# SinOncology/BreakID

Hardware: AMD Instinct MI355X
Metric: M reads/s clustered+split-scanned (higher is better)
Workload: dtype int32/u8 (+f64 sd replay)

## Files before the change

breakid_amd/csrc/lanes.hip:

```cpp
#include <algorithm>
#include <atomic>
#include <chrono>
#include <cmath>
#include <cstdio>
#include <numeric>
#include <thread>
#include <dirent.h>

#include "lanes.h"

static int g_hw_queues_at_init = 0;
void stage_set_hw_queues(int n) { g_hw_queues_at_init = n; }

static bool sort_service_on()
{
  static const bool on = !(getenv("BREAKID_SORT_SERVICE") && atoi(getenv("BREAKID_SORT_SERVICE")) == 0);
  return on;
}
constexpr int LANE_STREAMS_MAX = 4;
constexpr int SVC_STAGE_QUEUES = LANE_STREAMS_MAX + 3;
static bool lane_service(int fast) { return sort_service_on() && fast && g_hw_queues_at_init >= SVC_STAGE_QUEUES; }
static int stage_queues() { return std::max(1, g_hw_queues_at_init - 1); }
static int lanes_wanted(bool svc)
{
  const char *env = getenv("BREAKID_GROUP_LANES");
  static const int want_svc = env ? atoi(env) : 12;
  if (svc) return want_svc < 1 ? 1 : (want_svc > 26 ? 26 : want_svc);
  static const int want = env ? atoi(env) : std::min(4, stage_queues());
  return want < 1 ? 1 : (want > 26 ? 26 : want);
}
static bool lanes_apply(const StageInput &in, int fast)
{
  static const uint64_t min_pairs = getenv("BREAKID_LANES_MIN_PAIRS") ? strtoull(getenv("BREAKID_LANES_MIN_PAIRS"), nullptr, 10) : (1ull << 20);
  uint32_t large = 0;
  const uint64_t big = std::max<uint64_t>(2, min_pairs >> 6);
  for (uint32_t g = 0; g < in.jr.n_groups && g + 1 < in.gstart_host.size(); ++g) large += in.gstart_host[g + 1] - in.gstart_host[g] >= big ? 1u : 0u;
  const bool yes = lanes_wanted(lane_service(fast)) >= 2 && fast && in.jr.n_groups >= 4 && in.jr.n_pairs >= min_pairs && large >= 2;
  if (yes)
  {
    static bool told = false;
    const int K = lanes_wanted(lane_service(fast));
    if (!told && !lane_service(fast) && K > stage_queues() && bk_debug("lanes"))
    {
      told = true;
      fprintf(stderr, "[breakid] GPU_MAX_HW_QUEUES=%d: the lanes of chromosome-pair groups (bk_mask_and_cluster) and their heap kernels will share hardware queues "
                        "(BREAKID_GROUP_LANES=1: one pass)\n", g_hw_queues_at_init);
    }
  }
  return yes;
}

__global__ void k_svc_probe() {}
static int kfd_compute_queues(int device)
{
  char bus[64] = {0};
  if (hipDeviceGetPCIBusId(bus, (int) sizeof bus, device) != hipSuccess) return -1;
  unsigned dom = 0, b = 0, d = 0, f = 0;
  if (sscanf(bus, "%x:%x:%x.%x", &dom, &b, &d, &f) != 4) return -1;
  const unsigned long want_loc = (b << 8) | (d << 3) | f;
  auto read_file = [](const std::string &path, std::string &out) {
    FILE *fp = fopen(path.c_str(), "r");
    if (!fp) return false;
    char buf[4096];
    const size_t n = fread(buf, 1, sizeof buf - 1, fp);
    fclose(fp);
    buf[n] = 0;
    out = buf;
    return true;
  };
  auto list_dir = [](const std::string &path, std::vector<std::string> &names) {
    DIR *dp = opendir(path.c_str());
    if (!dp) return false;
    while (dirent *e = readdir(dp))
      if (e->d_name[0] != '.') names.push_back(e->d_name);
    closedir(dp);
    return true;
  };
  unsigned long gpu_id = 0;
  {
    std::vector<std::string> nodes;
    if (!list_dir("/sys/class/kfd/kfd/topology/nodes", nodes)) return -1;
    for (const std::string &n : nodes)
    {
      std::string props, id;
      const std::string base = "/sys/class/kfd/kfd/topology/nodes/" + n;
      if (!read_file(base + "/properties", props) || !read_file(base + "/gpu_id", id)) continue;
      unsigned long loc = ~0ul, domain = ~0ul;
      size_t p = props.find("location_id ");
      if (p != std::string::npos) loc = strtoul(props.c_str() + p + 12, nullptr, 10);
      p = props.find("domain ");
      if (p != std::string::npos) domain = strtoul(props.c_str() + p + 7, nullptr, 10);
      if (loc == want_loc && (domain == ~0ul || domain == dom) && strtoul(id.c_str(), nullptr, 10) != 0) gpu_id = strtoul(id.c_str(), nullptr, 10);
// ... 77 lines not shown
    cs.svc_late = 0;
    set(&cs.svc);
  }
  bool reachable(const std::vector<hipStream_t> &streams)
  {
    while (cs.svc_probe.size() < streams.size())
    {
      hipEvent_t e;
      HIP_CHECK(hipEventCreateWithFlags(&e, hipEventDisableTiming));
      cs.svc_probe.push_back(e);
    }
    for (size_t k = 0; k < streams.size(); ++k)
    {
      hipLaunchKernelGGL(k_svc_probe, dim3(1), dim3(64), 0, streams[k]);
      HIP_CHECK(hipEventRecord(cs.svc_probe[k], streams[k]));
    }
    const auto t0 = std::chrono::steady_clock::now();
    auto since = [&] { return std::chrono::duration<double>(std::chrono::steady_clock::now() - t0).count(); };
    bool ok = true;
    for (size_t k = 0; k < streams.size() && ok; ++k)
      for (;;)
      {
        const hipError_t e = hipEventQuery(cs.svc_probe[k]);
        if (e == hipSuccess) break;
        if (e != hipErrorNotReady) throw bk_error(BK_ERR_HIP, std::string("sort service probe: ") + hipGetErrorString(e));
        if (since() > 0.05)
        {
          ok = false;
          break;
        }
      }
    const double took = since();
    if (bk_debug("lanes")) fprintf(stderr, "[lanes] sort service probe: %zu streams in %.3f ms%s\n", streams.size(), took * 1e3, ok ? "" : " (gave up)");
    return ok && took < 0.003;
  }
  void set(SortService *s)
  {
    for (auto &l : cs.lanes)
    {
      l->cb.se.svc = s;
      l->cb.se.svc_slot = 0xFFFFFFFFu;
    }
  }
  void finish()
  {
    if (!on) return;
    on = false;
    set(nullptr);
    hipError_t e = hipStreamSynchronize(st);
    for (auto &l : cs.lanes)
      if (l->st && e == hipSuccess) e = hipStreamSynchronize(l->st);
    cs.svc.stop();
    device_turn.unlock();
    if (e != hipSuccess) throw bk_error(BK_ERR_HIP, std::string("sort service: ") + hipGetErrorString(e));
  }
  ~SvcStage()
  {
    try
    {
      finish();
    }
    catch (const bk_error &)
    {
    }
  }
};

static void snapshot_list(const PairList &L, DevBuf &idx, DevBuf *gof, DevBuf &goff, hipStream_t st)
{
  uint32_t *ii = idx.as<uint32_t>(L.n + 1), *ig = gof ? gof->as<uint32_t>(L.n + 1) : nullptr;
  uint64_t *io = goff.as<uint64_t>((uint64_t) L.ng + 1);
  if (L.n) HIP_CHECK(hipMemcpyAsync(ii, L.idx.get<uint32_t>(), L.n * 4, hipMemcpyDeviceToDevice, st));
  if (L.n && ig) HIP_CHECK(hipMemcpyAsync(ig, L.gof.get<uint32_t>(), L.n * 4, hipMemcpyDeviceToDevice, st));
  if (L.ng) HIP_CHECK(hipMemcpyAsync(io, L.goff.get<uint64_t>(), ((uint64_t) L.ng + 1) * 8, hipMemcpyDeviceToDevice, st));
}
static void cluster_list(const bk_pair *pairs, PairList &L, double w, int fast, DevBuf &cl, ClusterBufs &cb, AhcBufs &ab, hipStream_t st)
{
  if (fast)
    fast_cluster_all(pairs, L, w, cl, cb, st);
  else
    ahc_cluster_all(pairs, L, w, cl, ab, cb, st);
}

using LanePlan = std::vector<int>;
static LanePlan plan_owned(const StageInput &in)
{
  const uint32_t ng = in.jr.n_groups;
  const bool owned_only = !in.own_groups.empty();
  if (owned_only && in.own_groups.size() != ng) throw bk_error(BK_ERR_ARG, "bk_shard_own_groups: group count changed");
  LanePlan p(ng, 0);
  for (uint32_t g = 0; owned_only && g < ng; ++g)
    if (!in.own_groups[g]) p[g] = -1;
  return p;
}
static LanePlan plan_blind(const StageInput &in, int K)
{
  const uint32_t ng = in.jr.n_groups;
  std::vector<uint32_t> order(ng);
  std::iota(order.begin(), order.end(), 0u);
  auto size_of = [&](uint32_t g) { return in.gstart_host[g + 1] - in.gstart_host[g]; };
  std::stable_sort(order.begin(), order.end(), [&](uint32_t a, uint32_t b) { return size_of(a) > size_of(b); });
  constexpr double wexp = 2.0;
  LanePlan p = plan_owned(in);
  std::vector<double> load(K, 0.0);
  for (uint32_t i = 0; i < ng; ++i)
  {
    const uint32_t g = order[i];
    if (p[g] < 0) continue;
    int l = 0;
    for (int k = 1; k < K; ++k)
      if (load[k] < load[l]) l = k;
    load[l] += std::pow((double) size_of(g), wexp);
    p[g] = l;
  }
  return p;
}
static LanePlan plan_observed(const std::vector<uint64_t> &sizes, const std::vector<uint32_t> &hx, const std::vector<uint32_t> &hy, int K)
{
  const uint32_t ng = (uint32_t) sizes.size();
  constexpr double per_pair = 0.001;
  auto heap_cost = [](uint32_t m) { return (double) m + (m > 40947u ? 1.0 * (double) (m - 40947u) : 0.0); };
  std::vector<uint32_t> order(ng);
  std::iota(order.begin(), order.end(), 0u);
  auto chain = [&](uint32_t g) { return heap_cost(hx[g]) + heap_cost(hy[g]); };
  std::stable_sort(order.begin(), order.end(), [&](uint32_t a, uint32_t b) {
    const double ca = chain(a), cb = chain(b);
    return ca != cb ? ca > cb : sizes[a] > sizes[b];
  });
  LanePlan p(ng, 0);
  std::vector<double> mx(K, 0.0), my(K, 0.0), pairs(K, 0.0);
  auto cost = [&](int l) { return mx[l] + my[l] + per_pair * pairs[l]; };
  for (uint32_t g : order)
  {
    int best = 0;
    double best_cost = 0;
    for (int l = 0; l < K; ++l)
    {
      const double c = std::max(mx[l], heap_cost(hx[g])) + std::max(my[l], heap_cost(hy[g])) + per_pair * (pairs[l] + (double) sizes[g]);
      if (l == 0 || c < best_cost || (c == best_cost && cost(l) < cost(best)))
      {
        best = l;
        best_cost = c;
      }
    }
    mx[best] = std::max(mx[best], heap_cost(hx[g]));
    my[best] = std::max(my[best], heap_cost(hy[g]));
    pairs[best] += (double) sizes[g];
    p[g] = best;
  }
  if (bk_debug("lanes"))
    for (int l = 0; l < K; ++l)
    {
      fprintf(stderr, "[lanes] lane %d: max heap x %.0f y %.0f, %.0f pairs, cost %.0f; heavy groups:", l, mx[l], my[l], pairs[l], cost(l));
      for (uint32_t g = 0; g < ng; ++g)
        if (p[g] == l && (hx[g] || hy[g])) fprintf(stderr, " %u(%u,%u)", g, hx[g], hy[g]);
      fprintf(stderr, "\n");
    }
  return p;
}
static uint32_t *upload_drop(const LanePlan &p, int K, DevBuf &buf, hipStream_t st)
{
  const size_t row = p.size() + 1;
  std::vector<uint32_t> drop((size_t) K * row, 0u);
  for (int l = 0; l < K; ++l)
    for (size_t g = 0; g + 1 < row; ++g) drop[(size_t) l * row + g] = p[g] == l ? 0u : 1u;
  uint32_t *d = buf.as<uint32_t>(drop.size() + 1);
  HIP_CHECK(hipMemcpyAsync(d, drop.data(), drop.size() * 4, hipMemcpyHostToDevice, st));
  HIP_CHECK(hipStreamSynchronize(st));
  return d;
}

static void group_lanes(ClusterStage &cs, const StageInput &in, double w, int fast)
{
  const uint32_t ng = in.jr.n_groups;
  static const bool dbg = bk_debug("lanes");
  auto make_lanes = [&](int K, int S) {
    while ((int) cs.lanes.size() < K)
    {
      cs.lanes.emplace_back(new ClusterStage::Lane());
      cs.lanes.back()->cb.max_group_bound = cs.cb().max_group_bound;
    }
    for (int k = 1; k < S; ++k)
      if (!cs.lanes[k]->st) HIP_CHECK(hipStreamCreateWithFlags(&cs.lanes[k]->st, hipStreamNonBlocking));
  };
  bool use_svc = sort_service_on() && fast;
  if (use_svc && !lane_service(fast))
  {
    use_svc = false;
    tell_no_service();
    if (bk_debug("lanes")) fprintf(stderr, "[lanes] %d hardware queues, the sort service needs %d: not started\n", g_hw_queues_at_init, SVC_STAGE_QUEUES);
  }
  int K = lanes_wanted(use_svc);
  int S = use_svc ? std::max(1, std::min(LANE_STREAMS_MAX, K)) : K;
  make_lanes(K, S);
  std::vector<hipStream_t> stage_streams{in.st};
  for (int k = 1; k < S; ++k) stage_streams.push_back(cs.lanes[k]->st);
  SvcStage svc_stage(cs, in.device, in.st, use_svc, in.jr.n_pairs + 2ull * ng + 4096, cs.cb().max_group_bound, stage_streams);
  if (use_svc && !svc_stage.on)
  {
    use_svc = false;
    K = lanes_wanted(false);
    S = K;
    make_lanes(K, S);
  }
  if (!use_svc && bk_debug("lanes"))
  {
    fprintf(stderr, "[lanes] launch path: %d lanes, 1 stream each, %d hardware queues\n", K, g_hw_queues_at_init);
    fprintf(stderr, "[lanes] sorts as task dispatches on the lane streams\n");
  }
  auto lane = [&](int l) -> ClusterStage::Lane & { return *cs.lanes[l]; };
  auto lane_st = [&](int l) { const int k = l % S; return k == 0 ? in.st : cs.lanes[k]->st; };
  uint32_t *drop_base = nullptr;
  auto lane_drop = [&](int l) { return drop_base + (size_t) l * ((size_t) ng + 1); };
  std::vector<std::vector<uint8_t>> keep(K, std::vector<uint8_t>(ng, 0));
  auto upload_plan = [&](const LanePlan &p) {
    for (int l = 0; l < K; ++l)
      for (uint32_t g = 0; g < ng; ++g) keep[l][g] = p[g] == l ? 1 : 0;
    drop_base = upload_drop(p, K, cs.d_drop, in.st);
  };
  auto in_lanes = [&](auto body) {
    std::vector<std::string> err(K);
    std::vector<int> code(K, BK_OK);
    const auto t_start = std::chrono::steady_clock::now();
    auto guarded_body = [&](int l) {
      try
      {
        body(l);
        HIP_CHECK(hipStreamSynchronize(lane_st(l)));
        if (dbg)
          fprintf(stderr, "[lanes] lane %d done after %.2f ms\n", l, std::chrono::duration<double, std::milli>(std::chrono::steady_clock::now() - t_start).count());
      }
      catch (const bk_error &e)
      {
        code[l] = e.code;
        err[l] = e.msg;
      }
    };
    std::vector<std::thread> th;
    for (int l = 1; l < K; ++l)
      th.emplace_back([&, l] {
        (void) hipSetDevice(in.device);
        guarded_body(l);
      });
    guarded_body(0);
    for (std::thread &t : th) t.join();
    for (int l = 0; l < K; ++l)
      if (code[l] != BK_OK) throw bk_error(code[l], err[l]);
  };
  auto merge_all = [&](PairList ClusterStage::Lane::*which, PairList &out, DevBuf *cl_out) {
    std::vector<const PairList *> ls(K);
    std::vector<const uint32_t *> cls(K);
    for (int l = 0; l < K; ++l)
    {
      ls[l] = &(lane(l).*which);
      cls[l] = lane(l).d_cluster.get<uint32_t>();
    }
    merge_lists_many(ls.data(), cl_out ? cls.data() : nullptr, K, out, cl_out, in.st);
  };
  const bk_pair *pairs = in.jr.pairs;
  auto mask_lane = [&](int l, bool observe) {
    ClusterBufs &cb = lane(l).cb;
    if (observe)
    {
      cb.heavy_x.assign(ng, 0u);
      cb.heavy_y.assign(ng, 0u);
      cb.observe = true;
      cb.se.heavy_all = false;
    }
    remove_isolated_begin(pairs, in.jr.gof, in.jr.gstart, ng, in.jr.n_pairs, w, lane(l).list, cb, lane_st(l), lane_drop(l), in.gstart_host.data(), keep[l].data());
    if (observe) cb.heavy_x.assign(ng, 0u);
    remove_isolated_end(pairs, lane(l).list, cb, lane_st(l));
    if (observe) cb.observe = false;
  };
  auto cluster_lane = [&](int l) {
    PairList &L = lane(l).list, &iso = lane(l).iso;
    iso.n = L.n;
    iso.ng = L.ng;
    snapshot_list(L, iso.idx, &iso.gof, iso.goff, lane_st(l));
    cluster_list(pairs, L, w, fast, lane(l).d_cluster, lane(l).cb, cs.ab, lane_st(l));
  };
  const auto tp0 = std::chrono::steady_clock::now();
  auto phase = [&](const char *what) {
    if (dbg) fprintf(stderr, "[lanes] %s at %.2f ms\n", what, std::chrono::duration<double, std::milli>(std::chrono::steady_clock::now() - tp0).count());
  };
  upload_plan(plan_blind(in, K));
  phase("plan uploaded");
  if (use_svc)
    in_lanes([&](int l) {
      mask_lane(l, false);
      cluster_lane(l);
    });
  else
  {
    in_lanes([&](int l) { mask_lane(l, true); });
    PairList &mid = cs.lane_mid;
    merge_all(&ClusterStage::Lane::list, mid, nullptr);
    std::vector<uint64_t> goff_h((size_t) ng + 1);
    HIP_CHECK(hipMemcpyAsync(goff_h.data(), mid.goff.get<uint64_t>(), ((size_t) ng + 1) * 8, hipMemcpyDeviceToHost, in.st));
    HIP_CHECK(hipStreamSynchronize(in.st));
    std::vector<uint64_t> sizes(ng);
    std::vector<uint32_t> hx(ng, 0u), hy(ng, 0u);
    for (uint32_t g = 0; g < ng; ++g) sizes[g] = goff_h[g + 1] - goff_h[g];
    for (int l = 0; l < K; ++l)
      for (uint32_t g = 0; g < ng; ++g)
      {
        hx[g] = std::max(hx[g], lane(l).cb.heavy_x[g]);
        hy[g] = std::max(hy[g], lane(l).cb.heavy_y[g]);
      }
    upload_plan(plan_observed(sizes, hx, hy, K));
    in_lanes([&](int l) {
      list_subset_ranges(mid, goff_h.data(), keep[l].data(), lane(l).list, lane_st(l));
      cluster_lane(l);
    });
  }
  phase("lanes done");
  svc_stage.finish();
  phase("service stopped");
  if (use_svc && bk_debug("lanes")) fprintf(stderr, "[svc] tasks: %u wide, %u narrow\n", cs.svc.stats[0], cs.svc.stats[1]);
  PairList &iso_m = cs.lane_iso_m;
  merge_all(&ClusterStage::Lane::iso, iso_m, nullptr);
  merge_all(&ClusterStage::Lane::list, cs.list, &cs.d_cluster);
  HIP_CHECK(hipStreamSynchronize(in.st));
  phase("lists merged");
  cs.iso_n = iso_m.n;
  std::swap(cs.iso_idx, iso_m.idx);
  std::swap(cs.iso_goff, iso_m.goff);
}

void ClusterStage::run(const StageInput &in, double w, int fast)
{
  uint64_t mg = 0;
  for (uint32_t g = 0; g < in.jr.n_groups && g + 1 < in.gstart_host.size(); ++g) mg = std::max<uint64_t>(mg, in.gstart_host[g + 1] - in.gstart_host[g]);
  for (auto &l : lanes) l->cb.max_group_bound = mg;
  if (lanes_apply(in, fast))
  {
    in.timed("mask_and_cluster_lanes", [&] { group_lanes(*this, in, w, fast); });
    return;
  }
  SvcStage svc_stage(*this, in.device, in.st, true, in.jr.n_pairs + 2ull * in.jr.n_groups + 4096, cb().max_group_bound, {in.st});
  in.timed("remove_isolated", [&] {
    const uint32_t *drop = in.own_groups.empty() ? nullptr : upload_drop(plan_owned(in), 1, d_drop, in.st);
    remove_isolated_all(in.jr.pairs, in.jr.gof, in.jr.gstart, in.jr.n_groups, in.jr.n_pairs, w, list, cb(), in.st, drop);
  });
  iso_n = list.n;
  snapshot_list(list, iso_idx, nullptr, iso_goff, in.st);
  if (!fast) svc_stage.finish();
  in.timed(fast ? "fast_cluster" : "ahc_cluster", [&] { cluster_list(in.jr.pairs, list, w, fast, d_cluster, cb(), ab, in.st); });
  svc_stage.finish();
}

void ClusterStage::sort_forms(uint64_t out[3]) const
{
  out[0] = out[1] = out[2] = 0;
  for (const auto &l : lanes)
    for (int k = 0; k < 2; ++k) out[k] += l->cb.se.sorts[k];
}

void ClusterStage::debug_sort(int device, hipStream_t st, uint32_t *key, uint32_t *idx, const uint32_t *gof, const uint64_t *goff, uint32_t ng, uint64_t n, uint64_t max_group)
{
  SvcStage svc_stage(*this, device, st, true, n + 2ull * ng + 4096, max_group, {st});
  std_sort_groups(key, idx, gof, goff, ng, n, cb().se, st);
  svc_stage.finish();
}
```

breakid_amd/csrc/sortemu.h:

```cpp
#pragma once
#include "bk_common.h"
#include <vector>
#include <atomic>

struct SortService
{
  DevBuf ctl, slots[2], seq[2], jobs, dbg, pos[2];
  uint32_t pos_cap[2] = {0, 0};
  uint32_t cap[2] = {0, 0};
  hipStream_t st[2] = {nullptr, nullptr}, quit_stream = nullptr, st_copy = nullptr;
  uint32_t *quit_host = nullptr;
  uint32_t *quit_dev = nullptr;
  uint32_t cap32 = 0;
  uint32_t quit_word = 0, starts = 0;
  size_t wide_lds = 0;
  bool running = false;
  std::atomic<uint32_t> next_slot{0};
  uint32_t stats[8] = {};
  void start(uint64_t n_bound, uint64_t max_group, hipStream_t after);
  bool narrow_running(double seconds) const;
  void stop();
  uint32_t new_slot() { return next_slot.fetch_add(1u); }
  ~SortService();
  SortService() = default;
  SortService(const SortService &) = delete;
  SortService &operator=(const SortService &) = delete;
};

struct SortEmuBufs
{
  SortService *svc = nullptr;
  uint32_t svc_slot = 0xFFFFFFFFu, svc_epoch = 0;
  DevBuf heap_scratch, scratch32, scratch32b, rk_a, rk_b, chk_key0, chk_cnt, chk_bad;
  std::vector<uint32_t> *heavy = nullptr;
  bool heavy_all = false;
  DevBuf tj_ctl, tj_jobs, tj_slots[2], tj_seq[2], tj_pos[2], tj_heavy, tj_trace;
  uint32_t tj_cap[2] = {0, 0}, tj_epoch = 0;
  bool tj_ready = false;
  uint64_t sorts[2] = {0, 0};
  SortEmuBufs() = default;
  SortEmuBufs(const SortEmuBufs &) = delete;
  SortEmuBufs &operator=(const SortEmuBufs &) = delete;
};

void std_sort_groups(uint32_t *key, uint32_t *idx, const uint32_t *gof, const uint64_t *goff, uint32_t ng, uint64_t n, SortEmuBufs &b, hipStream_t st);
```

breakid_amd/csrc/sortemu.hip:

```cpp
#include "bk_common.h"
#include "sortemu.h"
#include <vector>
#include <mutex>
#include <algorithm>
#include <cstdio>
#include <chrono>
#include <thread>
#include <cstdlib>

namespace
{
typedef __attribute__((address_space(1))) uint32_t gu32_t;
__device__ __forceinline__ void st_through(uint32_t *p, uint32_t v) { __hip_atomic_store((gu32_t *) p, v, __ATOMIC_RELAXED, __HIP_MEMORY_SCOPE_AGENT); }
constexpr uint32_t FIN_MAX = 2048;
constexpr uint32_t HEAP_BIG_MIN = 4096;

typedef unsigned long long hent;
__device__ __forceinline__ uint32_t hkey(hent e) { return (uint32_t) (e >> 32); }

struct E64
{
  typedef hent T;
  static __device__ __forceinline__ uint32_t key(T e) { return (uint32_t) (e >> 32); }
};
struct E32
{
  typedef uint32_t T;
  static __device__ __forceinline__ uint32_t key(T e) { return e >> 16; }
};

template <class E> struct LdsMemT
{
  typedef typename E::T T;
  T *e;
  static __device__ __forceinline__ uint32_t key(T v) { return E::key(v); }
  __device__ __forceinline__ T ld(uint32_t i) const { return e[i]; }
  __device__ __forceinline__ void st(uint32_t i, T v) const { e[i] = v; }
  __device__ __forceinline__ void step_sync() const { __builtin_amdgcn_wave_barrier(); }
  __device__ __forceinline__ void launch_sync() const { __builtin_amdgcn_wave_barrier(); }
};
template <class E> struct GlbMemT
{
  typedef typename E::T T;
  T *e;
  static __device__ __forceinline__ uint32_t key(T v) { return E::key(v); }
  __device__ __forceinline__ T ld(uint32_t i) const { return e[i]; }
  __device__ __forceinline__ void st(uint32_t i, T v) const { e[i] = v; }
  __device__ __forceinline__ void step_sync() const { asm volatile("s_waitcnt vmcnt(0)" ::: "memory"); }
  __device__ __forceinline__ void launch_sync() const {}
};
typedef LdsMemT<E64> LdsMem;
typedef GlbMemT<E64> GlbMem;

template <class M> __device__ __forceinline__ bool sift_step(const M &mem, uint32_t &hole, uint32_t len, typename M::T v)
{
  typedef typename M::T T;
  const uint32_t right = 2 * (hole + 1), left = right - 1;
  T ec = 0;
  uint32_t c = 0;
  bool has = true;
  if (right < len)
  {
    const T el = mem.ld(left), er = mem.ld(right);
    if (M::key(er) < M::key(el))
    {
      c = left;
      ec = el;
    }
    else
    {
      c = right;
      ec = er;
    }
  }
  else if (left < len)
  {
    c = left;
    ec = mem.ld(left);
  }
  else
    has = false;
  if (has && !(M::key(ec) < M::key(v)))
  {
    mem.st(hole, ec);
// ... 962 lines not shown
        fprintf(stderr, "[svc]   %s workgroups by last state (1 polling, 5 took a task, 9 left):", kind ? "narrow" : "wide");
        for (auto &kv : hist) fprintf(stderr, " %u:%d", kv.first, kv.second);
        fprintf(stderr, "; first ones (state, polls, time of the last poll in 10 ns, how it left 6 error 7 quit 8 timeout):");
        for (uint32_t w = 0; w < 6 && w < n; ++w) fprintf(stderr, " [%u %u %u %u]", d[4 * (w + 4096 * kind)], d[4 * (w + 4096 * kind) + 1], d[4 * (w + 4096 * kind) + 2], d[4 * (w + 4096 * kind) + 3]);
        fprintf(stderr, "\n");
      }
    }
    uint32_t sq[4] = {};
    HIP_CHECK(hipMemcpy(sq, seq[1].get<uint32_t>(), sizeof sq, hipMemcpyDeviceToHost));
    fprintf(stderr, "[svc] tasks %u wide / %u narrow; workgroups started %u / %u, left on their own %u / %u, odd quit words read %u; error %u; wide queue head %u tail %u, narrow queue head %u tail %u (seq %u %u %u %u); job 0: remaining %u done %u heaps %u (longest %u)\n",
            stats[0], stats[1], stats[2], stats[3], stats[4], stats[5], stats[6], h[0], c[0], c[32], c[64], c[96], sq[0], sq[1], sq[2], sq[3], j0.remaining, j0.done, j0.n_heap, j0.max_heap);
  }
  if (h[0]) throw bk_error(h[0] & 2u ? BK_ERR_LIMIT : BK_ERR_HIP, "sort service: task error " + std::to_string(h[0]) + " (2 = ring overflow, 4 = a job timed out, 8 = a cut outside its segment, 16 = a task in the wrong queue, 32 = a node beyond the position lists, 64 = the finisher); first failing task: code " + std::to_string(h[8]) + ", " + std::to_string(h[9]) + " " + std::to_string(h[10]) + " " + std::to_string(h[11]));
}
SortService::~SortService()
{
  if (running)
  {
    running = false;
    if (quit_host && st_copy)
    {
      __atomic_store_n(quit_host, quit_word, __ATOMIC_SEQ_CST);
      (void) hipMemcpyAsync(ctl.get<uint32_t>() + 192, quit_host, 4, hipMemcpyHostToDevice, st_copy);
    }
    if (quit_stream) hipLaunchKernelGGL(k_svc_quit, dim3(1), dim3(1), 0, quit_stream, ctl.get<uint32_t>() + 192, quit_word);
    for (int k = 0; k < 2; ++k)
      if (st[k]) (void) hipStreamSynchronize(st[k]);
    DeferredFrees::end();
  }
  for (int k = 0; k < 2; ++k)
    if (st[k]) (void) hipStreamDestroy(st[k]);
  if (st_copy) (void) hipStreamDestroy(st_copy);
  if (quit_host) (void) hipHostFree(quit_host);
}

static void window_sorts(uint32_t *key, uint32_t *idx, const uint32_t *gof, uint32_t n, hipStream_t st);

static void std_sort_groups_svc(uint32_t *key, uint32_t *idx, const uint32_t *gof, const uint64_t *goff, uint32_t ng, uint32_t n, SortEmuBufs &b, hipStream_t st)
{
  SortService &S = *b.svc;
  if (b.svc_slot == 0xFFFFFFFFu)
  {
    b.svc_slot = S.new_slot();
    if (b.svc_slot >= SVC_MAX_JOBS) throw bk_error(BK_ERR_LIMIT, "sort service: more than 64 callers");
  }
  SvcJob d = {};
  d.key = key;
  d.idx = idx;
  d.hscratch = b.heap_scratch.as<hent>((uint64_t) n + HEAP_PAD);
  d.scratch32 = b.scratch32.as<uint32_t>((uint64_t) n + HEAP_PAD);
  d.scratch32b = b.scratch32b.as<uint32_t>((uint64_t) n + HEAP_PAD);
  d.rka = b.rk_a.as<unsigned long long>((uint64_t) n + HEAP_PAD);
  d.rkb = b.rk_b.as<unsigned long long>((uint64_t) n + HEAP_PAD);
  d.epoch = (b.svc_epoch++ % 0xFFFFFu) + 1u;
  const SvcParams P = svc_params(S);
  hipLaunchKernelGGL(k_svc_submit, dim3(1), dim3(256), 0, st, P, d, b.svc_slot, goff, ng);
  HIP_CHECK(hipGetLastError());
  {
    volatile const uint32_t *done = S.quit_host + SVC_H_DONE + b.svc_slot, *err = S.quit_host + SVC_H_ERROR;
    const auto t0 = std::chrono::steady_clock::now();
    for (uint32_t spins = 0; *done != d.epoch; ++spins)
    {
      if (*err != 0u)
        throw bk_error(BK_ERR_HIP, "sort service: a task failed (error " + std::to_string(*err) + "; first failing task: code " + std::to_string(err[1]) + ", " + std::to_string(err[2]) + " " + std::to_string(err[3]) + " " + std::to_string(err[4]) + ")");
      if ((spins & 1023u) == 1023u)
      {
        if (std::chrono::duration<double>(std::chrono::steady_clock::now() - t0).count() > 20.0) throw bk_error(BK_ERR_HIP, "sort service: a job did not finish");
        std::this_thread::yield();
      }
      else
        __builtin_ia32_pause();
    }
  }
  if (bk_debug("svc"))
  {
    SvcJob j;
    HIP_CHECK(hipMemcpy(&j, S.jobs.get<SvcJob>() + b.svc_slot, sizeof j, hipMemcpyDeviceToHost));
    fprintf(stderr, "[svc] slot %u sort %u: %u elements in %u groups; partitions and finisher done after %.3f ms, job after %.3f ms; %u elements in heaps, the longest %u, the heap that ended last %u elements in %.3f ms\n", b.svc_slot,
            b.svc_epoch, n, ng, (double) (j.t_parts - j.t_submit) * 1e-5, (double) (j.t_done - j.t_submit) * 1e-5, j.n_heap, j.max_heap, (uint32_t) j.last_heap, (double) (j.last_heap >> 32) * 1e-5);
  }
  window_sorts(key, idx, gof, n, st);
}

static void std_sort_groups_tasks(uint32_t *key, uint32_t *idx, const uint32_t *gof, const uint64_t *goff, uint32_t ng, uint32_t n, SortEmuBufs &b, hipStream_t st, const uint32_t *key0)
{
  static size_t dyn_lds = 0;
  static uint32_t cap32 = 0;
  static std::once_flag once;
  std::call_once(once, [] {
    const WideLds w = wide_lds_split(reinterpret_cast<const void *>(k_sort_job));
    dyn_lds = w.dyn_lds;
    cap32 = w.cap32;
    if (dyn_lds < SJ_TEAMS * SJ_TEAM_LDS) throw bk_error(BK_ERR_HIP, "k_sort_job: the narrow teams do not fit the LDS");
    HIP_CHECK(hipFuncSetAttribute(reinterpret_cast<const void *>(k_sort_job), hipFuncAttributeMaxDynamicSharedMemorySize, (int) dyn_lds));
  });
  std::vector<uint64_t> go((size_t) ng + 1);
  HIP_CHECK(hipMemcpyAsync(go.data(), goff, go.size() * 8, hipMemcpyDeviceToHost, st));
  HIP_CHECK(hipStreamSynchronize(st));
  uint64_t max_group = 0;
  for (uint32_t g = 0; g < ng; ++g) max_group = std::max<uint64_t>(max_group, go[g + 1] - go[g]);
  const uint32_t n_wide = std::min<uint32_t>(SJ_MAX_WIDE, std::max<uint32_t>(1, cdiv(n, 1u << 16)));
  const uint32_t n_narrow = std::min<uint32_t>(SJ_MAX_NARROW, std::max<uint32_t>(1, cdiv(n, 1u << 16)));
  SjParams S = {};
  SvcParams &P = S.P;
  {
    auto pow2 = [](uint64_t v) {
      uint32_t c = 1024;
      while (c < v && c < (1u << 30)) c <<= 1;
      return c;
    };
    const uint32_t want[2] = {pow2((uint64_t) n / HEAP_BIG_MIN + 4096), pow2((uint64_t) n / 16 + 4096)};
    for (int k = 0; k < 2; ++k)
      if (want[k] > b.tj_cap[k])
      {
        b.tj_cap[k] = want[k];
        b.tj_ready = false;
      }
    uint32_t *ctl = b.tj_ctl.as<uint32_t>(SJ_C_WORDS);
    for (int k = 0; k < 2; ++k)
    {
      P.q[k].head = ctl + 64 * k;
      P.q[k].tail = ctl + 64 * k + 32;
      P.q[k].slots = b.tj_slots[k].as<SvcTask>(b.tj_cap[k]);
      P.q[k].seq = b.tj_seq[k].as<uint32_t>(b.tj_cap[k]);
      P.q[k].mask = b.tj_cap[k] - 1;
      P.q[k].release = 1u;
    }
    P.error = ctl + SJ_C_ERROR;
    P.stats = ctl + SJ_C_STATS;
    P.quit_d = ctl + SJ_C_QUIT;
    P.host = ctl + SJ_C_HOST;
    P.jobs = b.tj_jobs.as<SvcJob>(SVC_MAX_JOBS);
    P.cap32 = cap32;
    P.quit_word = 0u;
    P.timeout_ticks = SJ_TIMEOUT_TICKS;
    P.pos_cap[0] = (uint32_t) std::max<uint64_t>(max_group, SVC_WIDE_MIN) + 64;
    P.pos_cap[1] = SVC_WIDE_MIN + 64;
    P.pos[0] = b.tj_pos[0].as<uint32_t>(2ull * P.pos_cap[0] * n_wide);
    P.pos[1] = b.tj_pos[1].as<uint32_t>(2ull * P.pos_cap[1] * n_narrow * SJ_TEAMS);
    P.dbg = nullptr;
    S.n_wide = n_wide;
    S.live = ctl + SJ_C_LIVE;
    S.gof = gof;
    S.heavy_min = b.heavy_all ? FIN_MAX : HEAP_RANKED_MIN;
    if (b.heavy)
    {
      S.heavy = b.tj_heavy.as<uint32_t>(ng);
      HIP_CHECK(hipMemsetAsync(S.heavy, 0, (size_t) ng * 4, st));
    }
  }
  static const bool dbg = bk_debug("svc");
  if (dbg) S.trace = b.tj_trace.as<unsigned long long>(8);
  if (!b.tj_ready)
  {
    HIP_CHECK(hipMemsetAsync(b.tj_ctl.p, 0, SJ_C_WORDS * 4, st));
    hipLaunchKernelGGL(k_svc_reset, dim3(cdiv(std::max(b.tj_cap[0], b.tj_cap[1]), 256)), dim3(256), 0, st, P);
    b.tj_ready = true;
  }
  SvcJob d = {};
  d.key = key;
  d.idx = idx;
  d.hscratch = b.heap_scratch.as<hent>((uint64_t) n + HEAP_PAD);
  d.scratch32 = b.scratch32.as<uint32_t>((uint64_t) n + HEAP_PAD);
  d.scratch32b = b.scratch32b.as<uint32_t>((uint64_t) n + HEAP_PAD);
  d.rka = b.rk_a.as<unsigned long long>((uint64_t) n + HEAP_PAD);
  d.rkb = b.rk_b.as<unsigned long long>((uint64_t) n + HEAP_PAD);
  d.epoch = (b.tj_epoch++ % 0xFFFFFu) + 1u;
  const SvcJobLds J = {d.key, d.idx, nullptr, nullptr, d.hscratch, d.scratch32, d.scratch32b, d.rka, d.rkb, P.jobs, d.epoch << 8};
  hipLaunchKernelGGL(k_sort_job_submit, dim3(1), dim3(256), 0, st, S, d, goff, ng);
  hipLaunchKernelGGL(k_sort_job, dim3(n_wide + n_narrow), dim3(1024), dyn_lds, st, S, J);
  HIP_CHECK(hipGetLastError());
  ++b.sorts[1];
  if (key0) sort_check("after the task dispatch", key, idx, key0, n, goff, ng, st, b);
  window_sorts(key, idx, gof, n, st);
  uint32_t h[16] = {};
  HIP_CHECK(hipMemcpyAsync(h, P.error, 12 * 4, hipMemcpyDeviceToHost, st));
  std::vector<uint32_t> hv;
  if (S.heavy)
  {
    hv.resize(ng);
    HIP_CHECK(hipMemcpyAsync(hv.data(), S.heavy, (size_t) ng * 4, hipMemcpyDeviceToHost, st));
  }
  unsigned long long tr[8] = {};
  if (S.trace) HIP_CHECK(hipMemcpyAsync(tr, S.trace, 5 * 8, hipMemcpyDeviceToHost, st));
  SvcJob j = {};
// ... 84 lines not shown
```

Measured before the change: 11710.

## Model lane sort costs to plan groups and scale narrow sort grids per lane

Replaces the greedy observed lane planner with a cost-model planner. It estimates each lane's sort time from heap chain length and partition work, places groups greedily, then improves the placement with local-search moves and swaps aimed at a lower worst-lane time. Each lane also gets a narrow-sort grid budget in proportion to its share of pairs, using the device CU count, so the narrow sort grids can grow past the old cap of 32. This is meant to balance the lanes and use idle CUs, at the cost of more host planning time and a risk of oversubscribing CUs when lanes run at the same time.

```diff
diff --git a/breakid_amd/csrc/lane_plan.h b/breakid_amd/csrc/lane_plan.h
--- /dev/null
+++ b/breakid_amd/csrc/lane_plan.h
@@ -0,0 +1,264 @@
+#pragma once
+#include <algorithm>
+#include <cmath>
+#include <cstdint>
+#include <cstdio>
+#include <numeric>
+#include <vector>
+
+using LanePlan = std::vector<int>;
+
+constexpr uint32_t SORT_GRID_BASE_MAX = 32;
+constexpr uint32_t SORT_GRID_MAX = 128;
+inline uint32_t sort_grid_base(uint64_t n) { return (uint32_t) std::min<uint64_t>(SORT_GRID_BASE_MAX, std::max<uint64_t>(1, (n + 65535) >> 16)); }
+inline uint32_t sort_grid_narrow(uint64_t n, uint32_t budget) { return std::max(sort_grid_base(n), std::min(SORT_GRID_MAX, budget)); }
+constexpr uint32_t LANE_CU_HEADROOM = 32;
+inline double lane_narrow_cus(uint32_t cus, int K)
+{
+  const double left = (double) cus - LANE_CU_HEADROOM - (double) SORT_GRID_BASE_MAX * K;
+  return left > 0.0 ? left : 0.0;
+}
+inline uint32_t lane_grid_budget(uint64_t n_lane, uint64_t n_total, uint32_t cus, int K)
+{
+  if (n_total == 0) return 0;
+  return (uint32_t) (lane_narrow_cus(cus, K) * (double) n_lane / (double) n_total);
+}
+
+inline LanePlan plan_blind(const std::vector<uint64_t> &sizes, const LanePlan &owned, int K)
+{
+  const uint32_t ng = (uint32_t) sizes.size();
+  std::vector<uint32_t> order(ng);
+  std::iota(order.begin(), order.end(), 0u);
+  std::stable_sort(order.begin(), order.end(), [&](uint32_t a, uint32_t b) { return sizes[a] > sizes[b]; });
+  constexpr double wexp = 2.0;
+  LanePlan p = owned;
+  std::vector<double> load(K, 0.0);
+  for (uint32_t i = 0; i < ng; ++i)
+  {
+    const uint32_t g = order[i];
+    if (p[g] < 0) continue;
+    int l = 0;
+    for (int k = 1; k < K; ++k)
+      if (load[k] < load[l]) l = k;
+    load[l] += std::pow((double) sizes[g], wexp);
+    p[g] = l;
+  }
+  return p;
+}
+
+struct LaneModel
+{
+  double pop_us = 0.18;
+  double spine_us = 1250.0;
+  double part_us_narrow = 0.0155;
+  double fixed_us = 1400.0, other_us = 0.00031;
+  uint32_t cus = 256;
+  int lanes = 3;
+
+  double sort_us(uint32_t longest, uint64_t n_lane, uint64_t n_total) const
+  {
+    const double share = n_total ? lane_narrow_cus(cus, lanes) * (double) n_lane / (double) n_total : 0.0;
+    const double narrow = std::max((double) sort_grid_base(n_lane), std::min((double) SORT_GRID_MAX, share));
+    return std::max(spine_us + pop_us * (double) longest, part_us_narrow * (double) n_lane / narrow);
+  }
+  double lane_us(uint32_t mx, uint32_t my, uint64_t n_lane, uint64_t n_total) const
+  {
+    if (n_lane == 0) return 0.0;
+    return sort_us(my, n_lane, n_total) + sort_us(mx, n_lane, n_total) + other_us * (double) n_lane + fixed_us;
+  }
+};
+
+struct LaneLoad
+{
+  uint32_t mx = 0, my = 0;
+  uint64_t n = 0;
+  double us = 0.0;
+};
+inline std::vector<LaneLoad> lane_loads(const LanePlan &p, const std::vector<uint64_t> &sizes, const std::vector<uint32_t> &hx, const std::vector<uint32_t> &hy, int K, const LaneModel &m)
+{
+  std::vector<LaneLoad> L(K);
+  uint64_t total = 0;
+  for (size_t g = 0; g < p.size(); ++g)
+  {
+    if (p[g] < 0) continue;
+    LaneLoad &l = L[p[g]];
+    l.mx = std::max(l.mx, hx[g]);
+    l.my = std::max(l.my, hy[g]);
+    l.n += sizes[g];
+    total += sizes[g];
+  }
+  for (LaneLoad &l : L) l.us = m.lane_us(l.mx, l.my, l.n, total);
+  return L;
+}
+
+inline LanePlan plan_observed(const std::vector<uint64_t> &sizes, const std::vector<uint32_t> &hx, const std::vector<uint32_t> &hy, const LanePlan &owned, int K, LaneModel m = LaneModel())
+{
+  constexpr int KMAX = 32;
+  const uint32_t ng = (uint32_t) sizes.size();
+  LanePlan p = owned;
+  K = std::max(1, std::min(K, KMAX));
+  m.lanes = K;
+  uint64_t total = 0;
+  std::vector<uint32_t> heavy, light;
+  for (uint32_t g = 0; g < ng; ++g)
+  {
+    if (p[g] < 0) continue;
+    p[g] = 0;
+    total += sizes[g];
+    ((hx[g] || hy[g]) ? heavy : light).push_back(g);
+  }
+  if (K == 1) return p;
+  auto chain = [&](uint32_t g) { return (uint64_t) hx[g] + hy[g]; };
+  std::stable_sort(heavy.begin(), heavy.end(), [&](uint32_t a, uint32_t b) {
+    const uint64_t ca = chain(a), cb = chain(b);
+    return ca != cb ? ca > cb : sizes[a] > sizes[b];
+  });
+  std::stable_sort(light.begin(), light.end(), [&](uint32_t a, uint32_t b) { return sizes[a] > sizes[b]; });
+  struct Times
+  {
+    double v[KMAX];
+  };
+  std::vector<uint8_t> is_heavy(ng, 0);
+  for (uint32_t g : heavy) is_heavy[g] = 1;
+  uint64_t n[KMAX] = {};
+  uint32_t mx[KMAX] = {}, my[KMAX] = {};
+  double us[KMAX] = {};
+  auto heaps_of = [&](int l) {
+    mx[l] = my[l] = 0;
+    for (uint32_t g : heavy)
+      if (p[g] == l)
+      {
+        mx[l] = std::max(mx[l], hx[g]);
+        my[l] = std::max(my[l], hy[g]);
+      }
+  };
+  auto profile = [&] {
+    Times t;
+    std::copy(us, us + K, t.v);
+    std::sort(t.v, t.v + K, std::greater<double>());
+    return t;
+  };
+  auto better = [&](const Times &a, const Times &b) {
+    for (int k = 0; k < K; ++k)
+      if (std::fabs(a.v[k] - b.v[k]) > 1e-6) return a.v[k] < b.v[k];
+    return false;
+  };
+  auto put = [&](uint32_t g, int l) {
+    n[l] += sizes[g];
+    p[g] = l;
+    if (is_heavy[g]) heaps_of(l);
+    us[l] = m.lane_us(mx[l], my[l], n[l], total);
+  };
+  auto take = [&](uint32_t g) {
+    const int l = p[g];
+    n[l] -= sizes[g];
+    p[g] = -2;
+    if (is_heavy[g]) heaps_of(l);
+    us[l] = m.lane_us(mx[l], my[l], n[l], total);
+  };
+  auto place = [&](uint32_t g) {
+    int best = 0;
+    Times best_t = {};
+    for (int l = 0; l < K; ++l)
+    {
+      put(g, l);
+      const Times t = profile();
+      take(g);
+      if (l == 0 || better(t, best_t))
+      {
+        best = l;
+        best_t = t;
+      }
+    }
+    put(g, best);
+  };
+  auto deal_light = [&] {
+    for (uint32_t g : light)
+      if (p[g] >= 0) take(g);
+    for (uint32_t g : light)
+    {
+      int best = 0;
+      double best_us = 0.0;
+      for (int l = 0; l < K; ++l)
+      {
+        const double t = m.lane_us(mx[l], my[l], n[l] + sizes[g], total);
+        if (l == 0 || t < best_us - 1e-6)
+        {
+          best = l;
+          best_us = t;
+        }
+      }
+      put(g, best);
+    }
+  };
+  Times now;
+  auto improves = [&] {
+    const Times t = profile();
+    if (!better(t, now)) return false;
+    now = t;
+    return true;
+  };
+  for (uint32_t g : heavy) p[g] = -2;
+  for (uint32_t g : light) p[g] = -2;
+  for (uint32_t g : heavy) place(g);
+  deal_light();
+  LanePlan best_p = p;
+  Times best_all = profile();
+  for (int outer = 0; outer < 4; ++outer)
+  {
+    now = profile();
+    for (int pass = 0; pass < 16; ++pass)
+    {
+      bool any = false;
+      for (uint32_t g : heavy)
+      {
+        const int from = p[g];
+        for (int l = 0; l < K && p[g] == from; ++l)
+        {
+          if (l == from) continue;
+          take(g);
+          put(g, l);
+          if (improves())
+            any = true;
+          else
+          {
+            take(g);
+            put(g, from);
+          }
+        }
+      }
+      for (size_t i = 0; i < heavy.size(); ++i)
+        for (size_t j = i + 1; j < heavy.size(); ++j)
+        {
+          const uint32_t a = heavy[i], b = heavy[j];
+          const int la = p[a], lb = p[b];
+          if (la == lb) continue;
+          take(a);
+          take(b);
+          put(a, lb);
+          put(b, la);
+          if (improves())
+            any = true;
+          else
+          {
+            take(a);
+            take(b);
+            put(a, la);
+            put(b, lb);
+          }
+        }
+      if (!any) break;
+    }
+    auto keep_if_better = [&] {
+      const Times t = profile();
+      if (!better(t, best_all)) return false;
+      best_all = t;
+      best_p = p;
+      return true;
+    };
+    keep_if_better();
+    deal_light();
+    if (!keep_if_better()) break;
+  }
+  return best_p;
+}
diff --git a/breakid_amd/csrc/lanes.hip b/breakid_amd/csrc/lanes.hip
--- a/breakid_amd/csrc/lanes.hip
+++ b/breakid_amd/csrc/lanes.hip
@@ -8,6 +8,7 @@
 #include <dirent.h>
 
 #include "lanes.h"
+#include "lane_plan.h"
 
 static int g_hw_queues_at_init = 0;
 void stage_set_hw_queues(int n) { g_hw_queues_at_init = n; }
@@ -251,7 +252,6 @@
     ahc_cluster_all(pairs, L, w, cl, ab, cb, st);
 }
 
-using LanePlan = std::vector<int>;
 static LanePlan plan_owned(const StageInput &in)
 {
   const uint32_t ng = in.jr.n_groups;
@@ -262,70 +262,32 @@
     if (!in.own_groups[g]) p[g] = -1;
   return p;
 }
-static LanePlan plan_blind(const StageInput &in, int K)
-{
-  const uint32_t ng = in.jr.n_groups;
-  std::vector<uint32_t> order(ng);
-  std::iota(order.begin(), order.end(), 0u);
-  auto size_of = [&](uint32_t g) { return in.gstart_host[g + 1] - in.gstart_host[g]; };
-  std::stable_sort(order.begin(), order.end(), [&](uint32_t a, uint32_t b) { return size_of(a) > size_of(b); });
-  constexpr double wexp = 2.0;
-  LanePlan p = plan_owned(in);
-  std::vector<double> load(K, 0.0);
-  for (uint32_t i = 0; i < ng; ++i)
-  {
-    const uint32_t g = order[i];
-    if (p[g] < 0) continue;
-    int l = 0;
-    for (int k = 1; k < K; ++k)
-      if (load[k] < load[l]) l = k;
-    load[l] += std::pow((double) size_of(g), wexp);
-    p[g] = l;
-  }
-  return p;
-}
-static LanePlan plan_observed(const std::vector<uint64_t> &sizes, const std::vector<uint32_t> &hx, const std::vector<uint32_t> &hy, int K)
-{
-  const uint32_t ng = (uint32_t) sizes.size();
-  constexpr double per_pair = 0.001;
-  auto heap_cost = [](uint32_t m) { return (double) m + (m > 40947u ? 1.0 * (double) (m - 40947u) : 0.0); };
-  std::vector<uint32_t> order(ng);
-  std::iota(order.begin(), order.end(), 0u);
-  auto chain = [&](uint32_t g) { return heap_cost(hx[g]) + heap_cost(hy[g]); };
-  std::stable_sort(order.begin(), order.end(), [&](uint32_t a, uint32_t b) {
-    const double ca = chain(a), cb = chain(b);
-    return ca != cb ? ca > cb : sizes[a] > sizes[b];
-  });
-  LanePlan p(ng, 0);
-  std::vector<double> mx(K, 0.0), my(K, 0.0), pairs(K, 0.0);
-  auto cost = [&](int l) { return mx[l] + my[l] + per_pair * pairs[l]; };
-  for (uint32_t g : order)
-  {
-    int best = 0;
-    double best_cost = 0;
-    for (int l = 0; l < K; ++l)
-    {
-      const double c = std::max(mx[l], heap_cost(hx[g])) + std::max(my[l], heap_cost(hy[g])) + per_pair * (pairs[l] + (double) sizes[g]);
-      if (l == 0 || c < best_cost || (c == best_cost && cost(l) < cost(best)))
-      {
-        best = l;
-        best_cost = c;
-      }
-    }
-    mx[best] = std::max(mx[best], heap_cost(hx[g]));
-    my[best] = std::max(my[best], heap_cost(hy[g]));
-    pairs[best] += (double) sizes[g];
-    p[g] = best;
-  }
-  if (bk_debug("lanes"))
-    for (int l = 0; l < K; ++l)
-    {
-      fprintf(stderr, "[lanes] lane %d: max heap x %.0f y %.0f, %.0f pairs, cost %.0f; heavy groups:", l, mx[l], my[l], pairs[l], cost(l));
-      for (uint32_t g = 0; g < ng; ++g)
-        if (p[g] == l && (hx[g] || hy[g])) fprintf(stderr, " %u(%u,%u)", g, hx[g], hy[g]);
-      fprintf(stderr, "\n");
-    }
-  return p;
+static std::vector<uint64_t> group_sizes(const StageInput &in)
+{
+  std::vector<uint64_t> sizes(in.jr.n_groups);
+  for (uint32_t g = 0; g < in.jr.n_groups; ++g) sizes[g] = in.gstart_host[g + 1] - in.gstart_host[g];
+  return sizes;
+}
+static uint32_t device_cus(int device)
+{
+  int cus = 0;
+  if (hipDeviceGetAttribute(&cus, hipDeviceAttributeMultiprocessorCount, device) != hipSuccess || cus < 1) return 0;
+  return (uint32_t) cus;
+}
+static void tell_plan(const LanePlan &p, const std::vector<uint64_t> &sizes, const std::vector<uint32_t> &hx, const std::vector<uint32_t> &hy, int K, const LaneModel &m, double plan_ms)
+{
+  const std::vector<LaneLoad> L = lane_loads(p, sizes, hx, hy, K, m);
+  uint64_t total = 0;
+  for (const LaneLoad &l : L) total += l.n;
+  fprintf(stderr, "[lanes] part 2 dealt in %.3f ms of the host\n", plan_ms);
+  for (int l = 0; l < K; ++l)
+  {
+    fprintf(stderr, "[lanes] lane %d: max heap x %u y %u, %llu pairs, sorts on %u wide + %u narrow workgroups, model %.2f ms; heavy groups:", l, L[l].mx, L[l].my, (unsigned long long) L[l].n,
+            sort_grid_base(L[l].n), sort_grid_narrow(L[l].n, lane_grid_budget(L[l].n, total, m.cus, K)), L[l].us * 1e-3);
+    for (size_t g = 0; g < p.size(); ++g)
+      if (p[g] == l && (hx[g] || hy[g])) fprintf(stderr, " %zu(%u,%u)", g, hx[g], hy[g]);
+    fprintf(stderr, "\n");
+  }
 }
 static uint32_t *upload_drop(const LanePlan &p, int K, DevBuf &buf, hipStream_t st)
 {
@@ -452,7 +414,34 @@
   auto phase = [&](const char *what) {
     if (dbg) fprintf(stderr, "[lanes] %s at %.2f ms\n", what, std::chrono::duration<double, std::milli>(std::chrono::steady_clock::now() - tp0).count());
   };
-  upload_plan(plan_blind(in, K));
+  LaneModel model;
+  model.cus = device_cus(in.device);
+  model.lanes = K;
+  struct BudgetsOff
+  {
+    ClusterStage &cs;
+    ~BudgetsOff()
+    {
+      for (auto &l : cs.lanes) l->cb.se.grid_budget = 0;
+    }
+  } budgets_off{cs};
+  auto set_budgets = [&](const LanePlan &p, const std::vector<uint64_t> &sizes) {
+    std::vector<uint64_t> n(K, 0);
+    uint64_t total = 0;
+    for (uint32_t g = 0; g < ng; ++g)
+      if (p[g] >= 0)
+      {
+        n[p[g]] += sizes[g];
+        total += sizes[g];
+      }
+    for (int l = 0; l < K; ++l) lane(l).cb.se.grid_budget = use_svc ? 0u : lane_grid_budget(n[l], total, model.cus, K);
+  };
+  {
+    const std::vector<uint64_t> sizes = group_sizes(in);
+    const LanePlan blind = plan_blind(sizes, plan_owned(in), K);
+    set_budgets(blind, sizes);
+    upload_plan(blind);
+  }
   phase("plan uploaded");
   if (use_svc)
     in_lanes([&](int l) {
@@ -476,7 +465,11 @@
         hx[g] = std::max(hx[g], lane(l).cb.heavy_x[g]);
         hy[g] = std::max(hy[g], lane(l).cb.heavy_y[g]);
       }
-    upload_plan(plan_observed(sizes, hx, hy, K));
+    const auto t_plan = std::chrono::steady_clock::now();
+    const LanePlan observed = plan_observed(sizes, hx, hy, plan_owned(in), K, model);
+    if (bk_debug("lanes")) tell_plan(observed, sizes, hx, hy, K, model, std::chrono::duration<double, std::milli>(std::chrono::steady_clock::now() - t_plan).count());
+    set_budgets(observed, sizes);
+    upload_plan(observed);
     in_lanes([&](int l) {
       list_subset_ranges(mid, goff_h.data(), keep[l].data(), lane(l).list, lane_st(l));
       cluster_lane(l);
diff --git a/breakid_amd/csrc/sortemu.h b/breakid_amd/csrc/sortemu.h
--- a/breakid_amd/csrc/sortemu.h
+++ b/breakid_amd/csrc/sortemu.h
@@ -37,6 +37,7 @@
   DevBuf tj_ctl, tj_jobs, tj_slots[2], tj_seq[2], tj_pos[2], tj_heavy, tj_trace;
   uint32_t tj_cap[2] = {0, 0}, tj_epoch = 0;
   bool tj_ready = false;
+  uint32_t grid_budget = 0;
   uint64_t sorts[2] = {0, 0};
   SortEmuBufs() = default;
   SortEmuBufs(const SortEmuBufs &) = delete;
diff --git a/breakid_amd/csrc/sortemu.hip b/breakid_amd/csrc/sortemu.hip
--- a/breakid_amd/csrc/sortemu.hip
+++ b/breakid_amd/csrc/sortemu.hip
@@ -1,5 +1,6 @@
 #include "bk_common.h"
 #include "sortemu.h"
+#include "lane_plan.h"
 #include <vector>
 #include <mutex>
 #include <algorithm>
@@ -1128,6 +1129,21 @@
   window_sorts(key, idx, gof, n, st);
 }
 
+constexpr uint64_t SORT_POS_BYTES_MAX = 256ull << 20;
+struct SortGridForce
+{
+  bool on;
+  uint32_t wide, narrow, min_n;
+};
+static SortGridForce sort_grid_force()
+{
+  SortGridForce f = {false, 0, 0, 0};
+  const char *env = getenv("BREAKID_SORT_GRID");
+  unsigned w = 0, nn = 0, mn = 0;
+  if (env && sscanf(env, "%u,%u,%u", &w, &nn, &mn) >= 2)
+    f = {true, std::min(std::max(w, 1u), SORT_GRID_MAX), std::min(std::max(nn, 1u), SORT_GRID_MAX), mn};
+  return f;
+}
 static void std_sort_groups_tasks(uint32_t *key, uint32_t *idx, const uint32_t *gof, const uint64_t *goff, uint32_t ng, uint32_t n, SortEmuBufs &b, hipStream_t st, const uint32_t *key0)
 {
   static size_t dyn_lds = 0;
@@ -1145,8 +1161,19 @@
   HIP_CHECK(hipStreamSynchronize(st));
   uint64_t max_group = 0;
   for (uint32_t g = 0; g < ng; ++g) max_group = std::max<uint64_t>(max_group, go[g + 1] - go[g]);
-  const uint32_t n_wide = std::min<uint32_t>(SJ_MAX_WIDE, std::max<uint32_t>(1, cdiv(n, 1u << 16)));
-  const uint32_t n_narrow = std::min<uint32_t>(SJ_MAX_NARROW, std::max<uint32_t>(1, cdiv(n, 1u << 16)));
+  static_assert(SORT_GRID_BASE_MAX == SJ_MAX_WIDE && SORT_GRID_BASE_MAX == SJ_MAX_NARROW, "lane_plan.h models the grid without a budget");
+  uint32_t n_wide = sort_grid_base(n), n_narrow = sort_grid_narrow(n, b.grid_budget);
+  static const SortGridForce force = sort_grid_force();
+  if (force.on && n >= force.min_n)
+  {
+    n_wide = force.wide;
+    n_narrow = force.narrow;
+  }
+  {
+    const uint64_t per_wg = 8ull * (std::max<uint64_t>(max_group, SVC_WIDE_MIN) + 64);
+    const uint32_t fit = (uint32_t) std::min<uint64_t>(SORT_GRID_MAX, SORT_POS_BYTES_MAX / per_wg);
+    n_wide = std::min(n_wide, std::max(fit, std::min(n_wide, sort_grid_base(n))));
+  }
   SjParams S = {};
   SvcParams &P = S.P;
   {
```

Result: faster. 12050, median of 6 (+3.0%).
